# lakesoul-io/LakeSoul

Measured on AMD Instinct MI355X. Metric: mor_scan_rows_per_sec, higher is better.
Workload: dtype mixed(int64,float64,int32,float32); 1 GPU; model=hash-PK lakehouse table, merge-on-read scan, scenario=10M base + 10x2M upserts per GPU (reference BASELINE.md config), rows_base_per_gpu=10000000, upserts=10, rows_upsert_per_gpu=2000000, hash_buckets=16, batch=row-group<=250k, zstd(1), dict off, global_batch=10000000, parallelism=dp1 hash-bucket sharding + RCCL all-to-all exchange, device=cuda

## Files before the change

### csrc/cpp/module.cc

```cpp
#include <torch/extension.h>

#include <atomic>
#include <cstring>
#include <memory>
#include <map>
#include <mutex>
#include <thread>
#include <unordered_map>
#include <chrono>

#include "murmur3.h"
#include "parquet_file.h"
#include "read_unit.h"
#include "str_seg.h"
#include "str_walk.h"
#include "unit_desc.h"
#include "huf_par.h"
#include "zstd_dec.h"

namespace py = pybind11;
using namespace lakesoul;


struct DtypeInfo {
  int32_t physical;
// ... 1045 lines not shown
    auto c = std::make_unique<lszstd::HufParCtx>();
    std::unique_ptr<uint8_t[]> out(new uint8_t[(size_t)rs]);
    bool ok = lszstd::huf_par_decode(src, (int64_t)b.size(), out.get(), rs,
                                     (int)lanes, *c);
    if (!ok) return py::make_tuple(py::none(), c->rounds);
    return py::make_tuple(py::bytes((const char*)out.get(), (size_t)rs), c->rounds);
  }, py::arg("frame"), py::arg("lanes"), py::arg("rs"));
  m.def("hash_columns_cpu", &hash_columns_cpu);
  m.def("hash_string_column_cpu", &hash_string_column_cpu);
  m.def("bucket_ids_from_hashes", &bucket_ids_from_hashes);
  m.def("spark_hash_bytes", [](py::bytes b, int64_t seed) {
    std::string s = b;
    return (int64_t)spark_hash_bytes((const uint8_t*)s.data(), (int64_t)s.size(),
                                     (uint32_t)seed);
  });
}
```

### csrc/hip/hip_module.cc

```cpp
#include <torch/extension.h>

#include <hip/hip_runtime.h>

#include <c10/hip/HIPStream.h>

#include <atomic>

#include "../cpp/unit_desc.h"
#include "kernels.h"

namespace py = pybind11;

using namespace lakesoul;

static hipStream_t cur_stream() {
  return c10::hip::getCurrentHIPStream().stream();
}

#define CHECK_GPU(t) TORCH_CHECK((t).is_cuda(), #t " must be on GPU"); \
  TORCH_CHECK((t).is_contiguous(), #t " must be contiguous")

#define CHECK_GPU_NONEMPTY(t)                                   \
  if ((t).numel()) {                                            \
    TORCH_CHECK((t).is_cuda(), #t " must be on GPU");           \
// ... 73 lines not shown
                             const int64_t* pos, void* out, int64_t n,
                             hipStream_t stream) {
  if (es == 1)
    launch_scatter_valid<uint8_t>((const uint8_t*)dense, vmask, pos, (uint8_t*)out, n, stream);
  else if (es == 2)
    launch_scatter_valid<uint16_t>((const uint16_t*)dense, vmask, pos, (uint16_t*)out, n, stream);
  else if (es == 4)
    launch_scatter_valid<uint32_t>((const uint32_t*)dense, vmask, pos, (uint32_t*)out, n, stream);
  else if (es == 8)
    launch_scatter_valid<uint64_t>((const uint64_t*)dense, vmask, pos, (uint64_t*)out, n, stream);
  else
    TORCH_CHECK(false, "scatter_valid: unsupported elem size ", es);
}


static std::pair<torch::Tensor, torch::Tensor> merge_key_streams(
    std::vector<torch::Tensor> keys) {
  TORCH_CHECK(!keys.empty(), "merge_sorted_keys: no streams");
  std::vector<torch::Tensor> rows;
  int64_t base = 0;
  for (auto& k : keys) {
    CHECK_GPU(k);
    TORCH_CHECK(k.scalar_type() == torch::kInt64 && k.dim() == 1,
                "merge_sorted_keys: keys must be 1-d int64");
    rows.push_back(torch::arange(base, base + k.numel(), k.options()));
    base += k.numel();
  }
  auto stream = cur_stream();
  while (keys.size() > 1) {
    std::vector<torch::Tensor> nk, nr;
    for (size_t j = 0; j + 1 < keys.size(); j += 2) {
      int64_t nA = keys[j].numel(), nB = keys[j + 1].numel();
      auto kO = torch::empty({nA + nB}, keys[j].options());
      auto vO = torch::empty({nA + nB}, keys[j].options());
      if (nA + nB)
        launch_merge_pairs(
            (const uint64_t*)keys[j].data_ptr(), (const uint64_t*)rows[j].data_ptr(), nA,
            (const uint64_t*)keys[j + 1].data_ptr(), (const uint64_t*)rows[j + 1].data_ptr(), nB,
            (uint64_t*)kO.data_ptr(), (uint64_t*)vO.data_ptr(), stream);
      nk.push_back(kO);
      nr.push_back(vO);
    }
    if (keys.size() % 2) {
      nk.push_back(keys.back());
      nr.push_back(rows.back());
    }
    keys = std::move(nk);
    rows = std::move(nr);
  }
  return {keys[0], rows[0]};
}

static torch::Tensor group_start_mask(torch::Tensor keys) {
  CHECK_GPU(keys);
  int64_t n = keys.numel();
  auto out = torch::empty({n}, keys.options().dtype(torch::kUInt8));
  launch_group_start((const uint64_t*)keys.data_ptr(), out.data_ptr<uint8_t>(), n,
                     cur_stream());
  return out;
}

static torch::Tensor pack_key_i64(torch::Tensor x) {
  CHECK_GPU(x);
  auto out = torch::empty_like(x);
  launch_pack_key_i64(x.data_ptr<int64_t>(), (uint64_t*)out.data_ptr(), x.numel(),
// ... 26 lines not shown
      bool wide = col.dim() == 2;
      int64_t es = col.element_size() * (wide ? col.size(1) : 1);
      TORCH_CHECK(es == 1 || es == 2 || es == 4 || es == 8,
                  "gather_fixed: unsupported elem size ", es);
      auto out = wide ? torch::empty({n, col.size(1)}, col.options())
                      : torch::empty({n}, col.options());
      tbl.src[tbl.ncols] = col.data_ptr();
      tbl.dst[tbl.ncols] = out.data_ptr();
      tbl.esize[tbl.ncols] = (int)es;
      tbl.ncols++;
      outs.push_back(out);
    }
    launch_gather_fixed_multi(tbl, idx.data_ptr<int64_t>(), n, cur_stream());
  }
  return outs;
}

static std::pair<torch::Tensor, torch::Tensor> take_strings(
    torch::Tensor bytes, torch::Tensor offsets, torch::Tensor idx) {
  CHECK_GPU_NONEMPTY(bytes);
  CHECK_GPU(offsets);
  CHECK_GPU(idx);
  TORCH_CHECK(offsets.scalar_type() == torch::kInt64 && offsets.numel() >= 1 &&
                  idx.scalar_type() == torch::kInt64,
              "take_strings: offsets (rows + 1) and idx must be int64");
  int64_t n = idx.numel(), nrows = offsets.numel() - 1;
  auto lens = offsets.narrow(0, 1, nrows) - offsets.narrow(0, 0, nrows);
  auto new_offs = torch::zeros({n + 1}, offsets.options());
  new_offs.narrow(0, 1, n).copy_(at::cumsum(lens.index({idx}), 0));
  int64_t total = n ? new_offs[n].item<int64_t>() : 0;
// ... 438 lines not shown
static py::list decode_unit(torch::Tensor vals, torch::Tensor validity_buf,
                            torch::Tensor dicts, torch::Tensor runs,
                            torch::Tensor soffs, torch::Tensor desc,
                            int64_t nfiles, int64_t ncols,
                            c10::optional<torch::Tensor> enc) {
  std::vector<UnitCol> cols;
  {
    py::gil_scoped_release rel;
    cols = decode_unit_cols(vals, validity_buf, dicts, runs, soffs, desc,
                            nfiles, ncols, enc_or_empty(enc));
  }
  return unit_cols_to_py(cols);
}

static std::vector<UnitCol> concat_unit_files(const std::vector<UnitCol>& flat,
                                              const torch::Tensor& desc,
                                              int64_t nfiles, int64_t ncols) {
  auto da = desc.accessor<int64_t, 2>();
  std::vector<UnitCol> out((size_t)ncols);
  for (int64_t c = 0; c < ncols; c++) {
    auto part = [&](int64_t f) -> const UnitCol& { return flat[(size_t)(f * ncols + c)]; };
    auto cat = [&](auto piece) {
      std::vector<torch::Tensor> parts;
      for (int64_t f = 0; f < nfiles; f++) parts.push_back(piece(f));
      return nfiles == 1 ? parts[0] : at::cat(parts, 0);
    };
    UnitCol& o = out[(size_t)c];
    o.present = true;
    o.is_string = part(0).is_string;
    torch::Tensor a_valid;
    for (int64_t f = 0; f < nfiles; f++)
      if (part(f).validity.defined()) a_valid = part(f).validity;
    if (a_valid.defined())
      o.validity = cat([&](int64_t f) {
        auto& v = part(f).validity;
        return v.defined() ? v : torch::ones({da[f * ncols + c][UD_NUM_VALUES]}, a_valid.options());
      });
    if (!o.is_string) {
      int64_t es = da[c][UD_ESIZE];
      o.data = cat([&](int64_t f) { return part(f).data.view({-1, es}); });
      continue;
    }
    int64_t byte_base = 0;
    o.offsets = cat([&](int64_t f) {
      auto offs = part(f).offsets;
      if (f) offs = (offs + byte_base).narrow(0, 1, offs.numel() - 1);
      byte_base += part(f).bytes.numel();
      return offs;
    });
    o.bytes = cat([&](int64_t f) { return part(f).bytes; });
  }
  return out;
}

static std::vector<UnitCol> scan_unit_uselast_cols(
    const torch::Tensor& vals, const torch::Tensor& validity_buf,
    const torch::Tensor& dicts, const torch::Tensor& runs,
    const torch::Tensor& soffs, const torch::Tensor& desc, int64_t nfiles,
    int64_t ncols, int64_t pk_ci, int64_t pk_es, const torch::Tensor& enc) {
  TORCH_CHECK(nfiles >= 1 && pk_ci >= 0 && pk_ci < ncols && (pk_es == 4 || pk_es == 8),
              "scan_unit_uselast: bad pk column");
  auto flat = decode_unit_cols(vals, validity_buf, dicts, runs, soffs, desc,
                               nfiles, ncols, enc);
  for (auto& c : flat)
    TORCH_CHECK(c.present && !c.is_list,
                "scan_unit_uselast: absent or list column (fallback)");

  std::vector<torch::Tensor> file_keys;
  for (int64_t f = 0; f < nfiles; f++) {
    auto& pk = flat[(size_t)(f * ncols + pk_ci)].data;
    file_keys.push_back(pack_key_i64(
        pk_es == 8 ? pk.view(torch::kInt64) : pk.view(torch::kInt32).to(torch::kInt64)));
  }
  auto [keys, order] = merge_key_streams(std::move(file_keys));

  int64_t n = keys.numel();
  auto keep = torch::empty({n}, keys.options().dtype(torch::kUInt8));
  launch_keep_last((const uint64_t*)keys.data_ptr(), keep.data_ptr<uint8_t>(), n,
                   cur_stream());
  auto src_idx = order.index({at::nonzero(keep).view(-1)});

  auto cols = concat_unit_files(flat, desc, nfiles, ncols);
  std::vector<torch::Tensor> fixed;
  for (auto& c : cols) {
    if (!c.is_string) fixed.push_back(c.data);
    if (c.validity.defined()) fixed.push_back(c.validity);
  }
  auto taken = gather_fixed(std::move(fixed), src_idx);
  size_t t = 0;
  for (auto& c : cols) {
    if (!c.is_string) c.data = taken[t++].view(-1);
    if (c.validity.defined()) c.validity = taken[t++];
    if (c.is_string)
      std::tie(c.offsets, c.bytes) = take_strings(c.bytes, c.offsets, src_idx);
  }
  return cols;
}

static py::list scan_unit_uselast(torch::Tensor vals, torch::Tensor validity_buf,
                                  torch::Tensor dicts, torch::Tensor runs,
                                  torch::Tensor soffs, torch::Tensor desc,
                                  int64_t nfiles, int64_t ncols, int64_t pk_ci,
                                  int64_t pk_es,
                                  c10::optional<torch::Tensor> enc) {
  std::vector<UnitCol> cols;
  {
    py::gil_scoped_release rel;
    cols = scan_unit_uselast_cols(vals, validity_buf, dicts, runs, soffs, desc,
                                  nfiles, ncols, pk_ci, pk_es, enc_or_empty(enc));
  }
// ... 204 lines not shown
  m.def("snappy_decompress_into", &snappy_decompress_into);
  m.def("lz4_decompress", &lz4_decompress);
  m.def("lz4_decompress_into", &lz4_decompress_into);
  m.def("scan_unit_uselast", &scan_unit_uselast, py::arg("vals"),
        py::arg("validity"), py::arg("dicts"), py::arg("runs"), py::arg("soffs"),
        py::arg("desc"), py::arg("nfiles"), py::arg("ncols"), py::arg("pk_ci"),
        py::arg("pk_es"), py::arg("enc") = py::none());
  m.def("decode_unit", &decode_unit, py::arg("vals"), py::arg("validity"),
        py::arg("dicts"), py::arg("runs"), py::arg("soffs"), py::arg("desc"),
        py::arg("nfiles"), py::arg("ncols"), py::arg("enc") = py::none());
  m.doc() = "lakesoul_amd gfx950 HIP kernels";
  m.def("hash_fixed_column", &hash_fixed_column);
  m.def("hash_string_column", &hash_string_column);
  m.def("bucket_ids", &bucket_ids);
  m.def("merge_sorted_keys", &merge_key_streams);
  m.def("group_start_mask", &group_start_mask);
  m.def("pack_key_i64", &pack_key_i64);
  m.def("pack_key_2xi32", &pack_key_2xi32);
  m.def("gather_fixed_multi", &gather_fixed);
  m.def("take_strings", &take_strings);
  m.def("gather_strings", &gather_strings);
  m.def("bytes_ne_mask", &bytes_ne_mask);
  m.def("segmented_sum", &segmented_sum);
  m.def("segmented_last", &segmented_last);
}
```

### csrc/hip/kernels.h

```cpp
#pragma once

#include <hip/hip_runtime.h>

#include <cstdint>

namespace lakesoul {

void launch_hash_fixed(int dt, const void* data, const uint8_t* validity,
                       const int64_t* prev, int64_t* out, int64_t n, int first,
                       hipStream_t s);
void launch_hash_string(const int32_t* offsets, const uint8_t* bytes,
                        const uint8_t* validity, const int64_t* prev,
                        int64_t* out, int64_t n, int first, hipStream_t s);
void launch_bucket_ids(const int64_t* hashes, int32_t* out, int64_t n,
                       uint32_t nb, hipStream_t s);

void launch_rle_expand(const uint8_t* payload, const int64_t* runs,
                       int64_t nruns, int32_t* out, int64_t n, hipStream_t s);
template <typename T>
void launch_dict_gather_scatter(const T* dict, const int32_t* idx,
                                const uint8_t* validity, const int64_t* pos,
                                T* out, int64_t n, hipStream_t s);
template <typename T>
void launch_scatter_valid(const T* dense, const uint8_t* validity,
                          const int64_t* pos, T* out, int64_t n, hipStream_t s);

void launch_merge_pairs(const uint64_t* kA, const uint64_t* vA, int64_t nA,
                        const uint64_t* kB, const uint64_t* vB, int64_t nB,
                        uint64_t* kOut, uint64_t* vOut, hipStream_t s);
void launch_keep_last(const uint64_t* keys, uint8_t* keep, int64_t n, hipStream_t s);
void launch_group_start(const uint64_t* keys, uint8_t* start, int64_t n, hipStream_t s);
void launch_pack_key_i64(const int64_t* x, uint64_t* out, int64_t n, hipStream_t s);
void launch_pack_key_2xi32(const int32_t* hi, const int32_t* lo, uint64_t* out,
                           int64_t n, hipStream_t s);

struct GatherTable {
  const void* src[16];
  void* dst[16];
  int esize[16];
  int ncols;
};
void launch_gather_fixed_multi(const GatherTable& tbl, const int64_t* idx,
                               int64_t n, hipStream_t s);
void launch_gather_strings(const uint8_t* src_bytes, const int64_t* src_off,
                           const int64_t* idx, const int64_t* dst_off,
                           uint8_t* dst_bytes, int64_t n, hipStream_t s);
void launch_bytes_ne_mask(const int64_t* offsets, const uint8_t* bytes,
                          const uint8_t* pattern, int plen, uint8_t* out,
                          int64_t n, hipStream_t s);

template <typename T, typename ACC>
void launch_segmented_sum(const T* vals, const int64_t* grp, const uint8_t* contrib,
                          const uint8_t* validity, ACC* out_sum,
                          int32_t* out_has_null, int64_t n, hipStream_t s);
void launch_segmented_last(const int64_t* grp, const uint8_t* contrib,
                           const uint8_t* validity, int64_t* out_idx, int64_t n,
                           hipStream_t s);

// ... 67 lines not shown
```

### csrc/hip/kernels.hip

```cpp

#include <hip/hip_runtime.h>

#include <cstdint>

#include "../cpp/murmur3.h"
#include "kernels.h"

namespace lakesoul {

#define LS_THREADS 256
#define LS_MAX_BLOCKS 2048

static inline int ls_blocks(int64_t n, int per_thread = 1) {
  int64_t b = (n + (int64_t)LS_THREADS * per_thread - 1) / ((int64_t)LS_THREADS * per_thread);
  if (b > LS_MAX_BLOCKS) b = LS_MAX_BLOCKS;
  if (b < 1) b = 1;
  return (int)b;
}


template <int DT>
__global__ void hash_fixed_kernel(const void* __restrict__ data,
                                  const uint8_t* __restrict__ validity,
                                  const int64_t* __restrict__ prev,
// ... 89 lines not shown
  }
}

template <typename T>
__global__ void scatter_valid_kernel(const T* __restrict__ dense,
                                     const uint8_t* __restrict__ validity,
                                     const int64_t* __restrict__ positions,
                                     T* __restrict__ out, int64_t n) {
  for (int64_t i = (int64_t)blockIdx.x * blockDim.x + threadIdx.x; i < n;
       i += (int64_t)gridDim.x * blockDim.x) {
    out[i] = validity[i] ? dense[positions[i]] : (T)0;
  }
}


__device__ inline int64_t merge_path_search(const uint64_t* A, int64_t nA,
                                            const uint64_t* B, int64_t nB,
                                            int64_t d) {
  int64_t lo = d > nB ? d - nB : 0;
  int64_t hi = d < nA ? d : nA;
  while (lo < hi) {
    int64_t mid = (lo + hi) >> 1;
    if (A[mid] <= B[d - mid - 1]) lo = mid + 1;
    else hi = mid;
  }
  return lo;
}

#define MERGE_VT 8
#define MERGE_TILE (LS_THREADS * MERGE_VT)

__global__ __launch_bounds__(LS_THREADS) void merge_pairs_kernel(
    const uint64_t* __restrict__ kA, const uint64_t* __restrict__ vA, int64_t nA,
    const uint64_t* __restrict__ kB, const uint64_t* __restrict__ vB, int64_t nB,
    uint64_t* __restrict__ kOut, uint64_t* __restrict__ vOut) {
  __shared__ uint64_t sk[MERGE_TILE + 2];
  __shared__ int64_t s_bounds[4];

  int64_t total = nA + nB;
  for (int64_t tile = blockIdx.x;; tile += gridDim.x) {
    int64_t d0 = tile * MERGE_TILE;
    if (d0 >= total) break;
    int64_t d1 = d0 + MERGE_TILE;
    if (d1 > total) d1 = total;

    if (threadIdx.x == 0) {
      s_bounds[0] = merge_path_search(kA, nA, kB, nB, d0);
      s_bounds[1] = merge_path_search(kA, nA, kB, nB, d1);
    }
    __syncthreads();
    int64_t a0 = s_bounds[0], a1 = s_bounds[1];
    int64_t b0 = d0 - a0, b1 = d1 - a1;
    int aCount = (int)(a1 - a0);
    int bCount = (int)(b1 - b0);

    for (int i = threadIdx.x; i < aCount; i += blockDim.x) sk[i] = kA[a0 + i];
    for (int i = threadIdx.x; i < bCount; i += blockDim.x)
      sk[aCount + i] = kB[b0 + i];
    __syncthreads();

    int local_d = threadIdx.x * MERGE_VT;
    int out_n = (int)(d1 - d0);
    if (local_d < out_n) {
      int lo = local_d > bCount ? local_d - bCount : 0;
      int hi = local_d < aCount ? local_d : aCount;
      while (lo < hi) {
        int mid = (lo + hi) >> 1;
        if (sk[mid] <= sk[aCount + local_d - mid - 1]) lo = mid + 1;
        else hi = mid;
      }
      int ai = lo;
      int bi = local_d - lo;
      int64_t base = d0 + local_d;
      int count = out_n - local_d < MERGE_VT ? out_n - local_d : MERGE_VT;
#pragma unroll
      for (int k = 0; k < MERGE_VT; k++) {
        if (k >= count) break;
        bool takeA;
        if (ai >= aCount) takeA = false;
        else if (bi >= bCount) takeA = true;
        else takeA = sk[ai] <= sk[aCount + bi];
        if (takeA) {
          kOut[base + k] = sk[ai];
          vOut[base + k] = vA[a0 + ai];
          ai++;
        } else {
          kOut[base + k] = sk[aCount + bi];
          vOut[base + k] = vB[b0 + bi];
          bi++;
        }
      }
    }
    __syncthreads();
  }
}

__global__ void keep_last_mask_kernel(const uint64_t* __restrict__ keys,
                                      uint8_t* __restrict__ keep, int64_t n) {
  for (int64_t i = (int64_t)blockIdx.x * blockDim.x + threadIdx.x; i < n;
       i += (int64_t)gridDim.x * blockDim.x) {
    keep[i] = (i == n - 1) || (keys[i] != keys[i + 1]);
  }
}

__global__ void group_start_mask_kernel(const uint64_t* __restrict__ keys,
                                        uint8_t* __restrict__ start, int64_t n) {
  for (int64_t i = (int64_t)blockIdx.x * blockDim.x + threadIdx.x; i < n;
       i += (int64_t)gridDim.x * blockDim.x) {
    start[i] = (i == 0) || (keys[i] != keys[i - 1]);
  }
}

__global__ void pack_key_i64_kernel(const int64_t* __restrict__ x,
                                    uint64_t* __restrict__ out, int64_t n) {
  for (int64_t i = (int64_t)blockIdx.x * blockDim.x + threadIdx.x; i < n;
       i += (int64_t)gridDim.x * blockDim.x) {
// ... 14 lines not shown


__global__ void gather_fixed_multi_kernel(GatherTable tbl,
                                          const int64_t* __restrict__ idx,
                                          int64_t n) {
  for (int64_t i = (int64_t)blockIdx.x * blockDim.x + threadIdx.x; i < n;
       i += (int64_t)gridDim.x * blockDim.x) {
    int64_t s = idx[i];
#pragma unroll 4
    for (int c = 0; c < tbl.ncols; c++) {
      switch (tbl.esize[c]) {
        case 1: ((uint8_t*)tbl.dst[c])[i] = ((const uint8_t*)tbl.src[c])[s]; break;
        case 2: ((uint16_t*)tbl.dst[c])[i] = ((const uint16_t*)tbl.src[c])[s]; break;
        case 4: ((uint32_t*)tbl.dst[c])[i] = ((const uint32_t*)tbl.src[c])[s]; break;
        default: ((uint64_t*)tbl.dst[c])[i] = ((const uint64_t*)tbl.src[c])[s]; break;
      }
    }
  }
}

__global__ void gather_strings_kernel(const uint8_t* __restrict__ src_bytes,
                                      const int64_t* __restrict__ src_offsets,
                                      const int64_t* __restrict__ idx,
                                      const int64_t* __restrict__ dst_offsets,
                                      uint8_t* __restrict__ dst_bytes,
                                      int64_t n) {
  int64_t waves_per_grid = ((int64_t)gridDim.x * blockDim.x) >> 6;
  int64_t wave = ((int64_t)blockIdx.x * blockDim.x + threadIdx.x) >> 6;
  int lane = threadIdx.x & 63;
  for (int64_t i = wave; i < n; i += waves_per_grid) {
// ... 117 lines not shown
template void launch_dict_gather_scatter<uint32_t>(const uint32_t*, const int32_t*, const uint8_t*, const int64_t*, uint32_t*, int64_t, hipStream_t);
template void launch_dict_gather_scatter<uint64_t>(const uint64_t*, const int32_t*, const uint8_t*, const int64_t*, uint64_t*, int64_t, hipStream_t);
template void launch_dict_gather_scatter<uint8_t>(const uint8_t*, const int32_t*, const uint8_t*, const int64_t*, uint8_t*, int64_t, hipStream_t);

template <typename T>
void launch_scatter_valid(const T* dense, const uint8_t* validity,
                          const int64_t* pos, T* out, int64_t n, hipStream_t s) {
  hipLaunchKernelGGL((scatter_valid_kernel<T>), dim3(ls_blocks(n)),
                     dim3(LS_THREADS), 0, s, dense, validity, pos, out, n);
}
template void launch_scatter_valid<uint8_t>(const uint8_t*, const uint8_t*, const int64_t*, uint8_t*, int64_t, hipStream_t);
template void launch_scatter_valid<uint16_t>(const uint16_t*, const uint8_t*, const int64_t*, uint16_t*, int64_t, hipStream_t);
template void launch_scatter_valid<uint32_t>(const uint32_t*, const uint8_t*, const int64_t*, uint32_t*, int64_t, hipStream_t);
template void launch_scatter_valid<uint64_t>(const uint64_t*, const uint8_t*, const int64_t*, uint64_t*, int64_t, hipStream_t);

void launch_merge_pairs(const uint64_t* kA, const uint64_t* vA, int64_t nA,
                        const uint64_t* kB, const uint64_t* vB, int64_t nB,
                        uint64_t* kOut, uint64_t* vOut, hipStream_t s) {
  int64_t ntiles = (nA + nB + MERGE_TILE - 1) / MERGE_TILE;
  int blocks = ntiles > LS_MAX_BLOCKS ? LS_MAX_BLOCKS : (int)ntiles;
  hipLaunchKernelGGL(merge_pairs_kernel, dim3(blocks), dim3(LS_THREADS), 0, s,
                     kA, vA, nA, kB, vB, nB, kOut, vOut);
}

void launch_keep_last(const uint64_t* keys, uint8_t* keep, int64_t n, hipStream_t s) {
  hipLaunchKernelGGL(keep_last_mask_kernel, dim3(ls_blocks(n)), dim3(LS_THREADS), 0, s,
                     keys, keep, n);
}

void launch_group_start(const uint64_t* keys, uint8_t* start, int64_t n, hipStream_t s) {
  hipLaunchKernelGGL(group_start_mask_kernel, dim3(ls_blocks(n)), dim3(LS_THREADS), 0, s,
                     keys, start, n);
}

void launch_pack_key_i64(const int64_t* x, uint64_t* out, int64_t n, hipStream_t s) {
  hipLaunchKernelGGL(pack_key_i64_kernel, dim3(ls_blocks(n)), dim3(LS_THREADS), 0, s,
                     x, out, n);
}

void launch_pack_key_2xi32(const int32_t* hi, const int32_t* lo, uint64_t* out,
                           int64_t n, hipStream_t s) {
  hipLaunchKernelGGL(pack_key_2xi32_kernel, dim3(ls_blocks(n)), dim3(LS_THREADS), 0, s,
                     hi, lo, out, n);
}

void launch_gather_fixed_multi(const GatherTable& tbl, const int64_t* idx,
                               int64_t n, hipStream_t s) {
  hipLaunchKernelGGL(gather_fixed_multi_kernel, dim3(ls_blocks(n)),
                     dim3(LS_THREADS), 0, s, tbl, idx, n);
}

void launch_gather_strings(const uint8_t* src_bytes, const int64_t* src_off,
                           const int64_t* idx, const int64_t* dst_off,
                           uint8_t* dst_bytes, int64_t n, hipStream_t s) {
  hipLaunchKernelGGL(gather_strings_kernel, dim3(ls_blocks(n, 1)),
                     dim3(LS_THREADS), 0, s, src_bytes, src_off, idx, dst_off,
                     dst_bytes, n);
}

void launch_bytes_ne_mask(const int64_t* offsets, const uint8_t* bytes,
                          const uint8_t* pattern, int plen, uint8_t* out,
                          int64_t n, hipStream_t s) {
  hipLaunchKernelGGL(bytes_ne_mask_kernel, dim3(ls_blocks(n)), dim3(LS_THREADS),
                     0, s, offsets, bytes, pattern, plen, out, n);
// ... 78 lines not shown
```

Baseline: 311.2 million rows/s.

## Fuse merge rounds with keep-last dedup and gather directly from per-file columns

Replaces the pairwise merge loop with a host-planned multi-pair round kernel that reads int32/int64 keys directly, using ping-pong buffers and no arange row tensors. The final round also applies keep-last deduplication in-kernel with a per-tile compaction, which removes the separate keep mask, nonzero and index step. Fixed-width and validity columns are then gathered straight from per-file parts through a file-lookup kernel, so the concat of all files is skipped. This cuts kernel launches, intermediate allocations and full-table copies, at the cost of more complex kernels and a per-row file search.

```diff
diff --git a/csrc/cpp/merge_plan.h b/csrc/cpp/merge_plan.h
--- /dev/null
+++ b/csrc/cpp/merge_plan.h
@@ -0,0 +1,91 @@
+#pragma once
+
+#include <cstdint>
+#include <vector>
+
+namespace lakesoul {
+
+constexpr int64_t MERGE_TILE_ROWS = 2048;
+constexpr int MP_INPUT = -1;
+constexpr int MP_RESULT = -2;
+
+struct MergeStream {
+  int buf = MP_INPUT;
+  int first = 0;
+  int count = 1;
+  int64_t off = 0;
+  int64_t n = 0;
+};
+
+struct MergePair {
+  MergeStream a, b;
+  int64_t first_tile = 0;
+  int64_t ntiles = 0;
+};
+
+struct MergeRound {
+  std::vector<MergePair> pairs;
+  bool has_carry = false;
+  MergeStream carry;
+  int buf_out = 0;
+  int64_t ntiles = 0;
+};
+
+struct MergePlan {
+  std::vector<MergeRound> rounds;
+  int nbufs = 0;
+  int64_t n = 0;
+};
+
+inline MergePlan plan_merge(const std::vector<int64_t>& lens) {
+  MergePlan plan;
+  std::vector<MergeStream> cur;
+  for (size_t i = 0; i < lens.size(); i++) {
+    MergeStream s;
+    s.first = (int)i;
+    s.off = plan.n;
+    s.n = lens[i];
+    plan.n += lens[i];
+    cur.push_back(s);
+  }
+  while (cur.size() > 1) {
+    MergeRound r;
+    bool last = cur.size() == 2;
+    if (last) {
+      r.buf_out = MP_RESULT;
+    } else {
+      bool used[3] = {false, false, false};
+      for (size_t j = 0; j < cur.size() - cur.size() % 2; j++)
+        if (cur[j].buf >= 0) used[cur[j].buf] = true;
+      r.buf_out = !used[0] ? 0 : !used[1] ? 1 : 2;
+      if (r.buf_out + 1 > plan.nbufs) plan.nbufs = r.buf_out + 1;
+    }
+    std::vector<MergeStream> next;
+    for (size_t j = 0; j + 1 < cur.size(); j += 2) {
+      MergePair p;
+      p.a = cur[j];
+      p.b = cur[j + 1];
+      p.first_tile = r.ntiles;
+      p.ntiles = (p.a.n + p.b.n + MERGE_TILE_ROWS - 1) / MERGE_TILE_ROWS;
+      r.ntiles += p.ntiles;
+      r.pairs.push_back(p);
+      MergeStream o;
+      o.buf = r.buf_out;
+      o.first = p.a.first;
+      o.count = p.a.count + p.b.count;
+      o.off = p.a.off;
+      o.n = p.a.n + p.b.n;
+      next.push_back(o);
+    }
+    if (cur.size() % 2) {
+      r.has_carry = true;
+      r.carry = cur.back();
+      next.push_back(cur.back());
+    }
+    plan.rounds.push_back(std::move(r));
+    cur = std::move(next);
+  }
+  return plan;
+}
+
+}
diff --git a/csrc/cpp/module.cc b/csrc/cpp/module.cc
--- a/csrc/cpp/module.cc
+++ b/csrc/cpp/module.cc
@@ -9,6 +9,7 @@
 #include <unordered_map>
 #include <chrono>
 
+#include "merge_plan.h"
 #include "murmur3.h"
 #include "parquet_file.h"
 #include "read_unit.h"
@@ -1084,4 +1085,19 @@
     return (int64_t)spark_hash_bytes((const uint8_t*)s.data(), (int64_t)s.size(),
                                      (uint32_t)seed);
   });
-}
+  m.def("merge_plan", [](std::vector<int64_t> lens) {
+    auto st = [](const MergeStream& s) {
+      return py::make_tuple(s.buf, s.first, s.count, s.off, s.n);
+    };
+    MergePlan plan = plan_merge(lens);
+    py::list rounds;
+    for (auto& r : plan.rounds) {
+      py::list pairs;
+      for (auto& p : r.pairs)
+        pairs.append(py::make_tuple(st(p.a), st(p.b), p.first_tile, p.ntiles));
+      rounds.append(py::make_tuple(pairs, r.has_carry ? py::object(st(r.carry)) : py::none(),
+                                   r.buf_out, r.ntiles));
+    }
+    return py::make_tuple(rounds, plan.nbufs, plan.n, MERGE_TILE_ROWS);
+  }, py::arg("lens"));
+}
diff --git a/csrc/hip/hip_module.cc b/csrc/hip/hip_module.cc
--- a/csrc/hip/hip_module.cc
+++ b/csrc/hip/hip_module.cc
@@ -6,6 +6,7 @@
 
 #include <atomic>
 
+#include "../cpp/merge_plan.h"
 #include "../cpp/unit_desc.h"
 #include "kernels.h"
 
@@ -111,41 +112,114 @@
 }
 
 
+static std::pair<torch::Tensor, torch::Tensor> merge_rounds(
+    const std::vector<torch::Tensor>& keys, int key_format, bool keep_last) {
+  auto stream = cur_stream();
+  auto i64 = keys[0].options().dtype(torch::kInt64);
+  std::vector<int64_t> lens;
+  for (auto& k : keys) lens.push_back(k.numel());
+  MergePlan plan = plan_merge(lens);
+  const int64_t n = plan.n;
+  if (keep_last && plan.rounds.empty()) {
+    MergeRound r;
+    MergePair p;
+    p.a.n = n;
+    p.b.off = n;
+    p.ntiles = (n + MERGE_TILE_ROWS - 1) / MERGE_TILE_ROWS;
+    r.pairs.push_back(p);
+    r.buf_out = MP_RESULT;
+    r.ntiles = p.ntiles;
+    plan.rounds.push_back(r);
+  }
+  torch::Tensor out_keys, out_rows, kbuf, rbuf, counts;
+  if (plan.nbufs) {
+    kbuf = torch::empty({plan.nbufs, n}, i64);
+    rbuf = torch::empty({plan.nbufs, n}, i64);
+  }
+  const int64_t last_tiles = plan.rounds.back().ntiles;
+  if (keep_last) {
+    out_rows = torch::empty({last_tiles * MERGE_TILE_ROWS}, i64);
+    counts = torch::empty({last_tiles}, i64);
+  } else {
+    out_keys = torch::empty({n}, i64);
+    out_rows = torch::empty({n}, i64);
+  }
+  auto set_stream = [&](const MergeStream& s, const void*& k, const int64_t*& r,
+                        int64_t& cnt, int64_t& base) {
+    cnt = s.n;
+    base = s.off;
+    if (s.buf == MP_INPUT) {
+      k = s.n ? keys[(size_t)s.first].data_ptr() : nullptr;
+      r = nullptr;
+    } else {
+      k = kbuf.data_ptr<int64_t>() + s.buf * n + s.off;
+      r = rbuf.data_ptr<int64_t>() + s.buf * n + s.off;
+    }
+  };
+  for (auto& round : plan.rounds) {
+    const bool last = round.buf_out == MP_RESULT;
+    for (size_t c0 = 0; c0 < round.pairs.size(); c0 += MERGE_PAIRS_PER_LAUNCH) {
+      MergeTable tbl;
+      tbl.npairs = 0;
+      tbl.ntiles = 0;
+      tbl.tile_counts = last && keep_last ? counts.data_ptr<int64_t>() : nullptr;
+      for (size_t j = c0; j < round.pairs.size() && tbl.npairs < MERGE_PAIRS_PER_LAUNCH; j++) {
+        const MergePair& p = round.pairs[j];
+        MergePairArg& a = tbl.p[tbl.npairs++];
+        set_stream(p.a, a.kA, a.rA, a.nA, a.baseA);
+        set_stream(p.b, a.kB, a.rB, a.nB, a.baseB);
+        if (last) {
+          a.kOut = keep_last ? nullptr : (uint64_t*)out_keys.data_ptr<int64_t>() + p.a.off;
+          a.rOut = out_rows.data_ptr<int64_t>() + p.a.off;
+        } else {
+          a.kOut = (uint64_t*)kbuf.data_ptr<int64_t>() + round.buf_out * n + p.a.off;
+          a.rOut = rbuf.data_ptr<int64_t>() + round.buf_out * n + p.a.off;
+        }
+        a.first_tile = tbl.ntiles;
+        tbl.ntiles += p.ntiles;
+      }
+      if (last && keep_last)
+        launch_merge_round_keep_last(tbl, key_format, stream);
+      else
+        launch_merge_round(tbl, key_format, stream);
+    }
+  }
+  if (!keep_last) return {out_keys, out_rows};
+  if (last_tiles == 0) return {out_keys, torch::empty({0}, i64)};
+  auto csum = at::cumsum(counts, 0);
+  int64_t kept = csum[last_tiles - 1].item<int64_t>();
+  auto src_idx = torch::empty({kept}, i64);
+  launch_compact_tiles(out_rows.data_ptr<int64_t>(), counts.data_ptr<int64_t>(),
+                       csum.data_ptr<int64_t>(), last_tiles,
+                       src_idx.data_ptr<int64_t>(), stream);
+  return {out_keys, src_idx};
+}
+
 static std::pair<torch::Tensor, torch::Tensor> merge_key_streams(
     std::vector<torch::Tensor> keys) {
   TORCH_CHECK(!keys.empty(), "merge_sorted_keys: no streams");
-  std::vector<torch::Tensor> rows;
-  int64_t base = 0;
   for (auto& k : keys) {
     CHECK_GPU(k);
     TORCH_CHECK(k.scalar_type() == torch::kInt64 && k.dim() == 1,
                 "merge_sorted_keys: keys must be 1-d int64");
-    rows.push_back(torch::arange(base, base + k.numel(), k.options()));
-    base += k.numel();
-  }
-  auto stream = cur_stream();
-  while (keys.size() > 1) {
-    std::vector<torch::Tensor> nk, nr;
-    for (size_t j = 0; j + 1 < keys.size(); j += 2) {
-      int64_t nA = keys[j].numel(), nB = keys[j + 1].numel();
-      auto kO = torch::empty({nA + nB}, keys[j].options());
-      auto vO = torch::empty({nA + nB}, keys[j].options());
-      if (nA + nB)
-        launch_merge_pairs(
-            (const uint64_t*)keys[j].data_ptr(), (const uint64_t*)rows[j].data_ptr(), nA,
-            (const uint64_t*)keys[j + 1].data_ptr(), (const uint64_t*)rows[j + 1].data_ptr(), nB,
-            (uint64_t*)kO.data_ptr(), (uint64_t*)vO.data_ptr(), stream);
-      nk.push_back(kO);
-      nr.push_back(vO);
-    }
-    if (keys.size() % 2) {
-      nk.push_back(keys.back());
-      nr.push_back(rows.back());
-    }
-    keys = std::move(nk);
-    rows = std::move(nr);
-  }
-  return {keys[0], rows[0]};
+  }
+  if (keys.size() == 1)
+    return {keys[0], torch::arange(keys[0].numel(), keys[0].options())};
+  return merge_rounds(keys, MERGE_KEY_PACKED, false);
+}
+
+static torch::Tensor unit_merge_src_idx(std::vector<torch::Tensor> keys) {
+  TORCH_CHECK(!keys.empty(), "unit_merge_src_idx: no streams");
+  auto dt = keys[0].scalar_type();
+  TORCH_CHECK(dt == torch::kInt64 || dt == torch::kInt32,
+              "unit_merge_src_idx: keys must be int64 or int32");
+  for (auto& k : keys) {
+    CHECK_GPU(k);
+    TORCH_CHECK(k.scalar_type() == dt && k.dim() == 1,
+                "unit_merge_src_idx: keys must be 1-d and of one dtype");
+  }
+  return merge_rounds(keys, dt == torch::kInt64 ? MERGE_KEY_I64 : MERGE_KEY_I32, true)
+      .second;
 }
 
 static torch::Tensor group_start_mask(torch::Tensor keys) {
@@ -202,6 +276,90 @@
     launch_gather_fixed_multi(tbl, idx.data_ptr<int64_t>(), n, cur_stream());
   }
   return outs;
+}
+
+struct FileColumn {
+  std::vector<const void*> src;
+  int es;
+  void* dst;
+};
+
+static void gather_files_launch(const std::vector<FileColumn>& cols,
+                                const std::vector<int64_t>& rows,
+                                const torch::Tensor& idx) {
+  const int64_t n = idx.numel();
+  const size_t nfiles = rows.size();
+  std::vector<int64_t> start(nfiles + 1, 0);
+  for (size_t f = 0; f < nfiles; f++) start[f + 1] = start[f] + rows[f];
+  for (size_t c0 = 0; c0 < cols.size(); c0 += GATHER_FILES_MAX_COLS) {
+    for (size_t f0 = 0; f0 < nfiles; f0 += GATHER_FILES_MAX_FILES) {
+      GatherFilesTable tbl = {};
+      tbl.nfiles = (int)std::min<size_t>(GATHER_FILES_MAX_FILES, nfiles - f0);
+      for (int f = 0; f <= tbl.nfiles; f++) tbl.start[f] = start[f0 + f];
+      for (int f = tbl.nfiles; f < GATHER_FILES_MAX_FILES; f++) tbl.start[f + 1] = tbl.start[f];
+      for (size_t c = c0; c < cols.size() && tbl.ncols < GATHER_FILES_MAX_COLS; c++) {
+        const FileColumn& col = cols[c];
+        TORCH_CHECK(col.es == 1 || col.es == 2 || col.es == 4 || col.es == 8,
+                    "gather_files: unsupported elem size ", col.es);
+        for (int f = 0; f < tbl.nfiles; f++) tbl.src[tbl.ncols][f] = col.src[f0 + f];
+        tbl.dst[tbl.ncols] = col.dst;
+        tbl.esize[tbl.ncols] = col.es;
+        tbl.ncols++;
+      }
+      launch_gather_files(tbl, idx.data_ptr<int64_t>(), n, cur_stream());
+    }
+  }
+}
+
+static std::vector<torch::Tensor> gather_files(
+    std::vector<std::vector<c10::optional<torch::Tensor>>> cols,
+    std::vector<int64_t> rows, torch::Tensor idx,
+    c10::optional<std::vector<torch::Tensor>> outs) {
+  CHECK_GPU(idx);
+  TORCH_CHECK(idx.scalar_type() == torch::kInt64 && idx.dim() == 1,
+              "gather_files: idx must be 1-d int64");
+  TORCH_CHECK(!outs.has_value() || outs->size() == cols.size(),
+              "gather_files: one output per column");
+  const int64_t n = idx.numel();
+  std::vector<FileColumn> fcs;
+  std::vector<torch::Tensor> res;
+  for (size_t c = 0; c < cols.size(); c++) {
+    TORCH_CHECK(cols[c].size() == rows.size(), "gather_files: one part per file");
+    FileColumn fc;
+    torch::Tensor first;
+    for (size_t f = 0; f < rows.size(); f++) {
+      if (!cols[c][f].has_value()) {
+        fc.src.push_back(nullptr);
+        continue;
+      }
+      const torch::Tensor& t = *cols[c][f];
+      CHECK_GPU(t);
+      if (!first.defined()) first = t;
+      TORCH_CHECK(t.dim() == 1 && t.numel() == rows[f] &&
+                      t.scalar_type() == first.scalar_type(),
+                  "gather_files: a part must be 1-d, of its file's row count "
+                  "and of the column's dtype");
+      fc.src.push_back(t.data_ptr());
+    }
+    TORCH_CHECK(first.defined(), "gather_files: a column of no parts");
+    fc.es = (int)first.element_size();
+    torch::Tensor out;
+    if (outs.has_value()) {
+      out = (*outs)[c];
+      CHECK_GPU(out);
+      TORCH_CHECK(out.dim() == 1 && out.numel() == n &&
+                      out.scalar_type() == first.scalar_type(),
+                  "gather_files: an output must be 1-d, of idx's size and of "
+                  "the column's dtype");
+    } else {
+      out = torch::empty({n}, first.options());
+    }
+    fc.dst = out.data_ptr();
+    fcs.push_back(std::move(fc));
+    res.push_back(out);
+  }
+  gather_files_launch(fcs, rows, idx);
+  return res;
 }
 
 static std::pair<torch::Tensor, torch::Tensor> take_strings(
@@ -670,9 +828,7 @@
 }
 
 static std::vector<UnitCol> concat_unit_files(const std::vector<UnitCol>& flat,
-                                              const torch::Tensor& desc,
                                               int64_t nfiles, int64_t ncols) {
-  auto da = desc.accessor<int64_t, 2>();
   std::vector<UnitCol> out((size_t)ncols);
   for (int64_t c = 0; c < ncols; c++) {
     auto part = [&](int64_t f) -> const UnitCol& { return flat[(size_t)(f * ncols + c)]; };
@@ -684,19 +840,7 @@
     UnitCol& o = out[(size_t)c];
     o.present = true;
     o.is_string = part(0).is_string;
-    torch::Tensor a_valid;
-    for (int64_t f = 0; f < nfiles; f++)
-      if (part(f).validity.defined()) a_valid = part(f).validity;
-    if (a_valid.defined())
-      o.validity = cat([&](int64_t f) {
-        auto& v = part(f).validity;
-        return v.defined() ? v : torch::ones({da[f * ncols + c][UD_NUM_VALUES]}, a_valid.options());
-      });
-    if (!o.is_string) {
-      int64_t es = da[c][UD_ESIZE];
-      o.data = cat([&](int64_t f) { return part(f).data.view({-1, es}); });
-      continue;
-    }
+    if (!o.is_string) continue;
     int64_t byte_base = 0;
     o.offsets = cat([&](int64_t f) {
       auto offs = part(f).offsets;
@@ -721,35 +865,57 @@
   for (auto& c : flat)
     TORCH_CHECK(c.present && !c.is_list,
                 "scan_unit_uselast: absent or list column (fallback)");
+  auto da = desc.accessor<int64_t, 2>();
 
   std::vector<torch::Tensor> file_keys;
+  std::vector<int64_t> rows;
   for (int64_t f = 0; f < nfiles; f++) {
     auto& pk = flat[(size_t)(f * ncols + pk_ci)].data;
-    file_keys.push_back(pack_key_i64(
-        pk_es == 8 ? pk.view(torch::kInt64) : pk.view(torch::kInt32).to(torch::kInt64)));
-  }
-  auto [keys, order] = merge_key_streams(std::move(file_keys));
-
-  int64_t n = keys.numel();
-  auto keep = torch::empty({n}, keys.options().dtype(torch::kUInt8));
-  launch_keep_last((const uint64_t*)keys.data_ptr(), keep.data_ptr<uint8_t>(), n,
-                   cur_stream());
-  auto src_idx = order.index({at::nonzero(keep).view(-1)});
-
-  auto cols = concat_unit_files(flat, desc, nfiles, ncols);
-  std::vector<torch::Tensor> fixed;
-  for (auto& c : cols) {
-    if (!c.is_string) fixed.push_back(c.data);
-    if (c.validity.defined()) fixed.push_back(c.validity);
-  }
-  auto taken = gather_fixed(std::move(fixed), src_idx);
-  size_t t = 0;
-  for (auto& c : cols) {
-    if (!c.is_string) c.data = taken[t++].view(-1);
-    if (c.validity.defined()) c.validity = taken[t++];
+    file_keys.push_back(pk.view(pk_es == 8 ? torch::kInt64 : torch::kInt32));
+    rows.push_back(file_keys.back().numel());
+  }
+  auto src_idx = unit_merge_src_idx(std::move(file_keys));
+  const int64_t n = src_idx.numel();
+
+  auto cols = concat_unit_files(flat, nfiles, ncols);
+  auto u8 = torch::TensorOptions().dtype(torch::kUInt8).device(vals.device());
+  std::vector<FileColumn> fcs;
+  for (int64_t c = 0; c < ncols; c++) {
+    auto part = [&](int64_t f) -> const UnitCol& { return flat[(size_t)(f * ncols + c)]; };
+    UnitCol& o = cols[(size_t)c];
+    if (!o.is_string) {
+      int64_t es = da[c][UD_ESIZE];
+      o.data = torch::empty({n * es}, u8);
+      FileColumn fc;
+      fc.es = (int)es;
+      fc.dst = o.data.data_ptr();
+      for (int64_t f = 0; f < nfiles; f++) {
+        TORCH_CHECK(part(f).data.numel() == rows[(size_t)f] * es,
+                    "scan_unit_uselast: a column's row count differs from the pk's");
+        fc.src.push_back(part(f).data.data_ptr());
+      }
+      fcs.push_back(std::move(fc));
+    }
+    bool any_valid = false;
+    for (int64_t f = 0; f < nfiles; f++) any_valid |= part(f).validity.defined();
+    if (any_valid) {
+      o.validity = torch::empty({n}, u8);
+      FileColumn fc;
+      fc.es = 1;
+      fc.dst = o.validity.data_ptr();
+      for (int64_t f = 0; f < nfiles; f++) {
+        auto& v = part(f).validity;
+        TORCH_CHECK(!v.defined() || v.numel() == rows[(size_t)f],
+                    "scan_unit_uselast: a validity's row count differs from the pk's");
+        fc.src.push_back(v.defined() ? v.data_ptr() : nullptr);
+      }
+      fcs.push_back(std::move(fc));
+    }
+  }
+  gather_files_launch(fcs, rows, src_idx);
+  for (auto& c : cols)
     if (c.is_string)
       std::tie(c.offsets, c.bytes) = take_strings(c.bytes, c.offsets, src_idx);
-  }
   return cols;
 }
 
@@ -984,6 +1150,9 @@
   m.def("hash_string_column", &hash_string_column);
   m.def("bucket_ids", &bucket_ids);
   m.def("merge_sorted_keys", &merge_key_streams);
+  m.def("unit_merge_src_idx", &unit_merge_src_idx, py::arg("keys"));
+  m.def("gather_files", &gather_files, py::arg("cols"), py::arg("rows"),
+        py::arg("idx"), py::arg("outs") = py::none());
   m.def("group_start_mask", &group_start_mask);
   m.def("pack_key_i64", &pack_key_i64);
   m.def("pack_key_2xi32", &pack_key_2xi32);
diff --git a/csrc/hip/kernels.h b/csrc/hip/kernels.h
--- a/csrc/hip/kernels.h
+++ b/csrc/hip/kernels.h
@@ -25,10 +25,31 @@
 void launch_scatter_valid(const T* dense, const uint8_t* validity,
                           const int64_t* pos, T* out, int64_t n, hipStream_t s);
 
-void launch_merge_pairs(const uint64_t* kA, const uint64_t* vA, int64_t nA,
-                        const uint64_t* kB, const uint64_t* vB, int64_t nB,
-                        uint64_t* kOut, uint64_t* vOut, hipStream_t s);
-void launch_keep_last(const uint64_t* keys, uint8_t* keep, int64_t n, hipStream_t s);
+constexpr int MERGE_PAIRS_PER_LAUNCH = 16;
+struct MergePairArg {
+  const void* kA;
+  const int64_t* rA;
+  int64_t nA, baseA;
+  const void* kB;
+  const int64_t* rB;
+  int64_t nB, baseB;
+  uint64_t* kOut;
+  int64_t* rOut;
+  int64_t first_tile;
+};
+struct MergeTable {
+  MergePairArg p[MERGE_PAIRS_PER_LAUNCH];
+  int npairs;
+  int64_t ntiles;
+  int64_t* tile_counts;
+};
+enum MergeKeyFormat { MERGE_KEY_I64 = 0, MERGE_KEY_I32 = 1, MERGE_KEY_PACKED = 2 };
+void launch_merge_round(const MergeTable& tbl, int key_format, hipStream_t s);
+void launch_merge_round_keep_last(const MergeTable& tbl, int key_format,
+                                  hipStream_t s);
+void launch_compact_tiles(const int64_t* slots, const int64_t* counts,
+                          const int64_t* csum, int64_t ntiles, int64_t* out,
+                          hipStream_t s);
 void launch_group_start(const uint64_t* keys, uint8_t* start, int64_t n, hipStream_t s);
 void launch_pack_key_i64(const int64_t* x, uint64_t* out, int64_t n, hipStream_t s);
 void launch_pack_key_2xi32(const int32_t* hi, const int32_t* lo, uint64_t* out,
@@ -42,6 +63,17 @@
 };
 void launch_gather_fixed_multi(const GatherTable& tbl, const int64_t* idx,
                                int64_t n, hipStream_t s);
+constexpr int GATHER_FILES_MAX_COLS = 16;
+constexpr int GATHER_FILES_MAX_FILES = 16;
+struct GatherFilesTable {
+  const void* src[GATHER_FILES_MAX_COLS][GATHER_FILES_MAX_FILES];
+  void* dst[GATHER_FILES_MAX_COLS];
+  int esize[GATHER_FILES_MAX_COLS];
+  int64_t start[GATHER_FILES_MAX_FILES + 1];
+  int ncols, nfiles;
+};
+void launch_gather_files(const GatherFilesTable& tbl, const int64_t* idx,
+                         int64_t n, hipStream_t s);
 void launch_gather_strings(const uint8_t* src_bytes, const int64_t* src_off,
                            const int64_t* idx, const int64_t* dst_off,
                            uint8_t* dst_bytes, int64_t n, hipStream_t s);
diff --git a/csrc/hip/kernels.hip b/csrc/hip/kernels.hip
--- a/csrc/hip/kernels.hip
+++ b/csrc/hip/kernels.hip
@@ -3,6 +3,7 @@
 
 #include <cstdint>
 
+#include "../cpp/merge_plan.h"
 #include "../cpp/murmur3.h"
 #include "kernels.h"
 
@@ -127,92 +128,187 @@
 }
 
 
-__device__ inline int64_t merge_path_search(const uint64_t* A, int64_t nA,
-                                            const uint64_t* B, int64_t nB,
-                                            int64_t d) {
+#define MERGE_VT 8
+#define MERGE_TILE (LS_THREADS * MERGE_VT)
+static_assert(MERGE_TILE == MERGE_TILE_ROWS, "tile size of the host plan");
+
+template <int KF>
+__device__ inline uint64_t merge_load_key(const void* k, bool raw, int64_t i) {
+  if constexpr (KF == MERGE_KEY_I64) {
+    if (raw) return (uint64_t)((const int64_t*)k)[i] ^ 0x8000000000000000ull;
+  } else if constexpr (KF == MERGE_KEY_I32) {
+    if (raw) return (uint64_t)((uint32_t)((const int32_t*)k)[i] ^ 0x80000000u);
+  }
+  return ((const uint64_t*)k)[i];
+}
+
+template <int KF>
+__device__ inline int64_t merge_path_search_wave(const void* A, bool rawA, int64_t nA,
+                                                 const void* B, bool rawB, int64_t nB,
+                                                 int64_t d, int lane) {
   int64_t lo = d > nB ? d - nB : 0;
   int64_t hi = d < nA ? d : nA;
   while (lo < hi) {
-    int64_t mid = (lo + hi) >> 1;
-    if (A[mid] <= B[d - mid - 1]) lo = mid + 1;
-    else hi = mid;
+    int64_t span = hi - lo;
+    int64_t mid = lo + ((span * lane) >> 6);
+    bool pred = merge_load_key<KF>(A, rawA, mid) <= merge_load_key<KF>(B, rawB, d - mid - 1);
+    int c = __popcll(__ballot(pred));
+    int64_t nlo = c > 0 ? lo + ((span * (c - 1)) >> 6) + 1 : lo;
+    int64_t nhi = c < 64 ? lo + ((span * c) >> 6) : hi;
+    lo = nlo;
+    hi = nhi;
   }
   return lo;
 }
 
-#define MERGE_VT 8
-#define MERGE_TILE (LS_THREADS * MERGE_VT)
-
-__global__ __launch_bounds__(LS_THREADS) void merge_pairs_kernel(
-    const uint64_t* __restrict__ kA, const uint64_t* __restrict__ vA, int64_t nA,
-    const uint64_t* __restrict__ kB, const uint64_t* __restrict__ vB, int64_t nB,
-    uint64_t* __restrict__ kOut, uint64_t* __restrict__ vOut) {
-  __shared__ uint64_t sk[MERGE_TILE + 2];
-  __shared__ int64_t s_bounds[4];
-
-  int64_t total = nA + nB;
-  for (int64_t tile = blockIdx.x;; tile += gridDim.x) {
-    int64_t d0 = tile * MERGE_TILE;
-    if (d0 >= total) break;
-    int64_t d1 = d0 + MERGE_TILE;
-    if (d1 > total) d1 = total;
-
-    if (threadIdx.x == 0) {
-      s_bounds[0] = merge_path_search(kA, nA, kB, nB, d0);
-      s_bounds[1] = merge_path_search(kA, nA, kB, nB, d1);
+template <int KF, bool KEEP_LAST>
+__global__ __launch_bounds__(LS_THREADS) void merge_round_kernel(MergeTable tbl) {
+  __shared__ uint64_t sk[MERGE_TILE + 4];
+  __shared__ int64_t sv[MERGE_TILE + 4];
+  __shared__ int64_t s_bounds[2];
+  __shared__ int s_wave_kept[LS_THREADS / 64];
+
+  const int lane = threadIdx.x & 63, wave = threadIdx.x >> 6;
+  for (int64_t tile = blockIdx.x; tile < tbl.ntiles; tile += gridDim.x) {
+    int j = 0;
+    while (j + 1 < tbl.npairs && tbl.p[j + 1].first_tile <= tile) j++;
+    const void* kA = tbl.p[j].kA;
+    const void* kB = tbl.p[j].kB;
+    const int64_t* rA = tbl.p[j].rA;
+    const int64_t* rB = tbl.p[j].rB;
+    const int64_t nA = tbl.p[j].nA, nB = tbl.p[j].nB;
+    const bool rawA = rA == nullptr, rawB = rB == nullptr;
+    const int64_t total = nA + nB;
+    const int64_t d0 = (tile - tbl.p[j].first_tile) * MERGE_TILE;
+    const int64_t d1 = d0 + MERGE_TILE < total ? d0 + MERGE_TILE : total;
+
+    if (wave < 2) {
+      int64_t a = merge_path_search_wave<KF>(kA, rawA, nA, kB, rawB, nB,
+                                             wave ? d1 : d0, lane);
+      if (lane == 0) s_bounds[wave] = a;
     }
     __syncthreads();
-    int64_t a0 = s_bounds[0], a1 = s_bounds[1];
-    int64_t b0 = d0 - a0, b1 = d1 - a1;
-    int aCount = (int)(a1 - a0);
-    int bCount = (int)(b1 - b0);
-
-    for (int i = threadIdx.x; i < aCount; i += blockDim.x) sk[i] = kA[a0 + i];
-    for (int i = threadIdx.x; i < bCount; i += blockDim.x)
-      sk[aCount + i] = kB[b0 + i];
+    const int64_t a0 = s_bounds[0], a1 = s_bounds[1];
+    const int64_t b0 = d0 - a0, b1 = d1 - a1;
+    const int aCount = (int)(a1 - a0), bCount = (int)(b1 - b0);
+    const int aExt = aCount + ((KEEP_LAST && a1 < nA) ? 1 : 0);
+    const int bExt = bCount + ((KEEP_LAST && b1 < nB) ? 1 : 0);
+
+    for (int i = threadIdx.x; i < aExt; i += LS_THREADS) {
+      sk[i] = merge_load_key<KF>(kA, rawA, a0 + i);
+      sv[i] = rawA ? tbl.p[j].baseA + a0 + i : rA[a0 + i];
+    }
+    for (int i = threadIdx.x; i < bExt; i += LS_THREADS) {
+      sk[aExt + i] = merge_load_key<KF>(kB, rawB, b0 + i);
+      sv[aExt + i] = rawB ? tbl.p[j].baseB + b0 + i : rB[b0 + i];
+    }
     __syncthreads();
 
-    int local_d = threadIdx.x * MERGE_VT;
-    int out_n = (int)(d1 - d0);
-    if (local_d < out_n) {
+    const int out_n = (int)(d1 - d0);
+    const int local_d = threadIdx.x * MERGE_VT;
+    int count = out_n - local_d;
+    count = count < 0 ? 0 : count > MERGE_VT ? MERGE_VT : count;
+    uint64_t ok[MERGE_VT];
+    int64_t ov[MERGE_VT];
+    int ai = 0, bi = 0;
+    if (count) {
       int lo = local_d > bCount ? local_d - bCount : 0;
       int hi = local_d < aCount ? local_d : aCount;
       while (lo < hi) {
         int mid = (lo + hi) >> 1;
-        if (sk[mid] <= sk[aCount + local_d - mid - 1]) lo = mid + 1;
+        if (sk[mid] <= sk[aExt + local_d - mid - 1]) lo = mid + 1;
         else hi = mid;
       }
-      int ai = lo;
-      int bi = local_d - lo;
-      int64_t base = d0 + local_d;
-      int count = out_n - local_d < MERGE_VT ? out_n - local_d : MERGE_VT;
+      ai = lo;
+      bi = local_d - lo;
+    }
+    uint64_t ka = sk[ai], kb = sk[aExt + bi];
+    int64_t va = sv[ai], vb = sv[aExt + bi];
+#pragma unroll
+    for (int k = 0; k < MERGE_VT; k++) {
+      if (k < count) {
+        bool takeA = bi >= bCount || (ai < aCount && ka <= kb);
+        if (takeA) {
+          ok[k] = ka;
+          ov[k] = va;
+          ai++;
+          ka = sk[ai];
+          va = sv[ai];
+        } else {
+          ok[k] = kb;
+          ov[k] = vb;
+          bi++;
+          kb = sk[aExt + bi];
+          vb = sv[aExt + bi];
+        }
+      }
+    }
+
+    if constexpr (!KEEP_LAST) {
+      __syncthreads();
 #pragma unroll
       for (int k = 0; k < MERGE_VT; k++) {
-        if (k >= count) break;
-        bool takeA;
-        if (ai >= aCount) takeA = false;
-        else if (bi >= bCount) takeA = true;
-        else takeA = sk[ai] <= sk[aCount + bi];
-        if (takeA) {
-          kOut[base + k] = sk[ai];
-          vOut[base + k] = vA[a0 + ai];
-          ai++;
-        } else {
-          kOut[base + k] = sk[aCount + bi];
-          vOut[base + k] = vB[b0 + bi];
-          bi++;
+        if (k < count) {
+          sk[local_d + k] = ok[k];
+          sv[local_d + k] = ov[k];
         }
       }
+      __syncthreads();
+      uint64_t* kOut = tbl.p[j].kOut + d0;
+      int64_t* rOut = tbl.p[j].rOut + d0;
+      for (int i = threadIdx.x; i < out_n; i += LS_THREADS) {
+        kOut[i] = sk[i];
+        rOut[i] = sv[i];
+      }
+    } else {
+      const bool hasA = ai < aExt, hasB = bi < bExt;
+      const uint64_t succ = hasA && hasB ? (ka <= kb ? ka : kb) : hasA ? ka : kb;
+      const bool has_succ = hasA || hasB;
+      unsigned keep = 0;
+#pragma unroll
+      for (int k = 0; k < MERGE_VT; k++) {
+        if (k < count) {
+          bool kp = k + 1 < count ? ok[k] != ok[k + 1] : (!has_succ || ok[k] != succ);
+          keep |= (unsigned)kp << k;
+        }
+      }
+      const int mine = __popc(keep);
+      int incl = mine;
+#pragma unroll
+      for (int o = 1; o < 64; o <<= 1) {
+        int up = __shfl_up(incl, o, 64);
+        if (lane >= o) incl += up;
+      }
+      if (lane == 63) s_wave_kept[wave] = incl;
+      __syncthreads();
+      int pos = incl - mine, tile_kept = 0;
+#pragma unroll
+      for (int w = 0; w < LS_THREADS / 64; w++) {
+        if (w < wave) pos += s_wave_kept[w];
+        tile_kept += s_wave_kept[w];
+      }
+#pragma unroll
+      for (int k = 0; k < MERGE_VT; k++) {
+        if (keep >> k & 1) sv[pos++] = ov[k];
+      }
+      __syncthreads();
+      int64_t* slot = tbl.p[j].rOut + d0;
+      for (int i = threadIdx.x; i < tile_kept; i += LS_THREADS) slot[i] = sv[i];
+      if (threadIdx.x == 0) tbl.tile_counts[tile] = tile_kept;
     }
     __syncthreads();
   }
 }
 
-__global__ void keep_last_mask_kernel(const uint64_t* __restrict__ keys,
-                                      uint8_t* __restrict__ keep, int64_t n) {
-  for (int64_t i = (int64_t)blockIdx.x * blockDim.x + threadIdx.x; i < n;
-       i += (int64_t)gridDim.x * blockDim.x) {
-    keep[i] = (i == n - 1) || (keys[i] != keys[i + 1]);
+__global__ void compact_tiles_kernel(const int64_t* __restrict__ slots,
+                                     const int64_t* __restrict__ counts,
+                                     const int64_t* __restrict__ csum,
+                                     int64_t ntiles, int64_t* __restrict__ out) {
+  for (int64_t tile = blockIdx.x; tile < ntiles; tile += gridDim.x) {
+    int64_t cnt = counts[tile];
+    const int64_t* src = slots + tile * MERGE_TILE;
+    int64_t* dst = out + (csum[tile] - cnt);
+    for (int64_t i = threadIdx.x; i < cnt; i += blockDim.x) dst[i] = src[i];
   }
 }
 
@@ -257,6 +353,36 @@
         case 2: ((uint16_t*)tbl.dst[c])[i] = ((const uint16_t*)tbl.src[c])[s]; break;
         case 4: ((uint32_t*)tbl.dst[c])[i] = ((const uint32_t*)tbl.src[c])[s]; break;
         default: ((uint64_t*)tbl.dst[c])[i] = ((const uint64_t*)tbl.src[c])[s]; break;
+      }
+    }
+  }
+}
+
+__global__ __launch_bounds__(LS_THREADS) void gather_files_kernel(
+    GatherFilesTable tbl, const int64_t* __restrict__ idx, int64_t n) {
+  __shared__ const void* s_src[GATHER_FILES_MAX_COLS * GATHER_FILES_MAX_FILES];
+  __shared__ int64_t s_start[GATHER_FILES_MAX_FILES + 1];
+  for (int i = threadIdx.x; i < GATHER_FILES_MAX_COLS * GATHER_FILES_MAX_FILES;
+       i += LS_THREADS)
+    s_src[i] = tbl.src[i / GATHER_FILES_MAX_FILES][i % GATHER_FILES_MAX_FILES];
+  if (threadIdx.x <= GATHER_FILES_MAX_FILES) s_start[threadIdx.x] = tbl.start[threadIdx.x];
+  __syncthreads();
+  const int nfiles = tbl.nfiles;
+  const int64_t lo = tbl.start[0], hi = tbl.start[nfiles];
+  for (int64_t i = (int64_t)blockIdx.x * blockDim.x + threadIdx.x; i < n;
+       i += (int64_t)gridDim.x * blockDim.x) {
+    int64_t s = idx[i];
+    if (s < lo || s >= hi) continue;
+    int f = 0;
+    for (int j = 1; j < nfiles; j++) f += s_start[j] <= s;
+    int64_t r = s - s_start[f];
+    for (int c = 0; c < tbl.ncols; c++) {
+      const void* p = s_src[c * GATHER_FILES_MAX_FILES + f];
+      switch (tbl.esize[c]) {
+        case 1: ((uint8_t*)tbl.dst[c])[i] = p ? ((const uint8_t*)p)[r] : (uint8_t)1; break;
+        case 2: ((uint16_t*)tbl.dst[c])[i] = p ? ((const uint16_t*)p)[r] : (uint16_t)1; break;
+        case 4: ((uint32_t*)tbl.dst[c])[i] = p ? ((const uint32_t*)p)[r] : 1u; break;
+        default: ((uint64_t*)tbl.dst[c])[i] = p ? ((const uint64_t*)p)[r] : 1ull; break;
       }
     }
   }
@@ -404,18 +530,33 @@
 template void launch_scatter_valid<uint32_t>(const uint32_t*, const uint8_t*, const int64_t*, uint32_t*, int64_t, hipStream_t);
 template void launch_scatter_valid<uint64_t>(const uint64_t*, const uint8_t*, const int64_t*, uint64_t*, int64_t, hipStream_t);
 
-void launch_merge_pairs(const uint64_t* kA, const uint64_t* vA, int64_t nA,
-                        const uint64_t* kB, const uint64_t* vB, int64_t nB,
-                        uint64_t* kOut, uint64_t* vOut, hipStream_t s) {
-  int64_t ntiles = (nA + nB + MERGE_TILE - 1) / MERGE_TILE;
-  int blocks = ntiles > LS_MAX_BLOCKS ? LS_MAX_BLOCKS : (int)ntiles;
-  hipLaunchKernelGGL(merge_pairs_kernel, dim3(blocks), dim3(LS_THREADS), 0, s,
-                     kA, vA, nA, kB, vB, nB, kOut, vOut);
-}
-
-void launch_keep_last(const uint64_t* keys, uint8_t* keep, int64_t n, hipStream_t s) {
-  hipLaunchKernelGGL(keep_last_mask_kernel, dim3(ls_blocks(n)), dim3(LS_THREADS), 0, s,
-                     keys, keep, n);
+template <bool KEEP_LAST>
+static void launch_merge_round_t(const MergeTable& tbl, int key_format, hipStream_t s) {
+  if (tbl.ntiles <= 0) return;
+  dim3 g(tbl.ntiles > LS_MAX_BLOCKS ? LS_MAX_BLOCKS : (int)tbl.ntiles), b(LS_THREADS);
+  switch (key_format) {
+    case MERGE_KEY_I64: hipLaunchKernelGGL((merge_round_kernel<MERGE_KEY_I64, KEEP_LAST>), g, b, 0, s, tbl); break;
+    case MERGE_KEY_I32: hipLaunchKernelGGL((merge_round_kernel<MERGE_KEY_I32, KEEP_LAST>), g, b, 0, s, tbl); break;
+    default: hipLaunchKernelGGL((merge_round_kernel<MERGE_KEY_PACKED, KEEP_LAST>), g, b, 0, s, tbl); break;
+  }
+}
+
+void launch_merge_round(const MergeTable& tbl, int key_format, hipStream_t s) {
+  launch_merge_round_t<false>(tbl, key_format, s);
+}
+
+void launch_merge_round_keep_last(const MergeTable& tbl, int key_format,
+                                  hipStream_t s) {
+  launch_merge_round_t<true>(tbl, key_format, s);
+}
+
+void launch_compact_tiles(const int64_t* slots, const int64_t* counts,
+                          const int64_t* csum, int64_t ntiles, int64_t* out,
+                          hipStream_t s) {
+  if (ntiles <= 0) return;
+  hipLaunchKernelGGL(compact_tiles_kernel,
+                     dim3(ntiles > LS_MAX_BLOCKS ? LS_MAX_BLOCKS : (int)ntiles),
+                     dim3(LS_THREADS), 0, s, slots, counts, csum, ntiles, out);
 }
 
 void launch_group_start(const uint64_t* keys, uint8_t* start, int64_t n, hipStream_t s) {
@@ -438,6 +579,13 @@
                                int64_t n, hipStream_t s) {
   hipLaunchKernelGGL(gather_fixed_multi_kernel, dim3(ls_blocks(n)),
                      dim3(LS_THREADS), 0, s, tbl, idx, n);
+}
+
+void launch_gather_files(const GatherFilesTable& tbl, const int64_t* idx,
+                         int64_t n, hipStream_t s) {
+  if (n <= 0) return;
+  hipLaunchKernelGGL(gather_files_kernel, dim3(ls_blocks(n)), dim3(LS_THREADS),
+                     0, s, tbl, idx, n);
 }
 
 void launch_gather_strings(const uint8_t* src_bytes, const int64_t* src_off,
```

Result: faster. 337.0 million rows/s (median of 6 runs) (+8.3%).
